# moberweger/deep-prior-pp

Measured on AMD Instinct MI355X. Metric: depth-crops/sec (NYU ResNet50 bs128) 1/2/4/8 GPU; mean 3D joint err (mm), higher is better.
Workload: dtype f32; 1 GPU; NYU posereg_embedding ResNet (type 0, 30-D PCA prior) train step: fused augment + fwd + bwd + ADAM, bs128/GPU fp32, 128x128x1 crops; global_batch=128, parallelism=dp1, augment=True, augment_pipelined=True, bn=local per-GPU batch statistics, launch_mode=native

## Files before the change

deep-prior-pp_amd/csrc/gemm_expand.hip:

```cpp
#include "gemm_args.h"

namespace {

template <int KT, bool BKC, bool IT2, bool ACT, bool RES, bool BNB, bool LZ = false, bool PB = false, bool ST = false>
__global__ __launch_bounds__(DPP_THREADS) DPP_WAVES_PER_EU(1, 2) void gemm_expand_kernel(GemmArgs ga, int rpw) {
    static_assert(!PB || ((KT % 32 == 0 || KT == 16) && !LZ), "bf16 MFMA operands: whole 32-deep steps, or K = 16 with a zero upper half");
    dpp_kernarg_warm<sizeof(GemmArgs)>();
    const dpp_gemm_desc& d = ga.d;
    constexpr int KL = KT / 4, KV = KL / 4;
    constexpr int RT = 2, RI = 16 * RT;
    const int lane = threadIdx.x & 63, l15 = lane & 15, kq = lane >> 4;
    const int NG = d.N >> 6, nblk = d.M / rpw;
    const int gw = blockIdx.x * 4 + (threadIdx.x >> 6);
    if (gw >= NG * nblk) return;
    const int cg = gw % NG, rblk = gw / NG;
    const int n0 = cg * 64 + 4 * l15;
    const int wrow0 = rblk * rpw, iters = rpw / RI;
    const dpp_epilogue& ep = d.epi;
    const int modeA = ACT ? d.actA.mode : 0;
    const bool relu_mask = BNB && ep.bn_relu != 0;
    const bool a16 = ST && !LZ && ga.shA != 0, c16 = ST && (d.store & DPP_ST_C) != 0, x16 = ST && (d.store & DPP_ST_BNX) != 0;
    dpp_stamp(ga.prof, 0);

    float bw[4][KL];
    if (BKC) {
#pragma unroll
        for (int ct = 0; ct < 4; ++ct)
#pragma unroll
            for (int j = 0; j < KV; ++j) {
                const float4 t = *reinterpret_cast<const float4*>(d.B + (size_t)(n0 + ct) * d.ldb + kq * KL + 4 * j);
                bw[ct][4 * j] = t.x; bw[ct][4 * j + 1] = t.y; bw[ct][4 * j + 2] = t.z; bw[ct][4 * j + 3] = t.w;
            }
    } else {
#pragma unroll
        for (int e = 0; e < KL; ++e) {
            const float4 t = *reinterpret_cast<const float4*>(d.B + (size_t)(kq * KL + e) * d.ldb + n0);
            bw[0][e] = t.x; bw[1][e] = t.y; bw[2][e] = t.z; bw[3][e] = t.w;
        }
    }
    constexpr int KS = PB ? (KL + 7) / 8 : 1;
    dpp_bf16x8 bwp[4][KS];
    if (PB) {
#pragma unroll
        for (int ct = 0; ct < 4; ++ct)
#pragma unroll
            for (int ss = 0; ss < KS; ++ss)
#pragma unroll
                for (int q = 0; q < 8; ++q) bwp[ct][ss][q] = (dpp_bf16)(ss * 8 + q < KL ? bw[ct][ss * 8 + q < KL ? ss * 8 + q : 0] : 0.0f);
    }
    struct Regs { float4 a[RT][KV]; float4 a2[RT][LZ ? KV : 1]; float4 res[RT][4]; float4 bx[RT][4]; };
    auto fetch = [&](Regs& g, int it) {
        const int r0 = wrow0 + it * RI;
#pragma unroll
        for (int rt = 0; rt < RT; ++rt) {
            const size_t oa = (size_t)(r0 + rt * 16 + l15) * d.lda + kq * KL;
            if (a16) {
#pragma unroll
                for (int j = 0; j < KV; ++j) g.a[rt][j] = dpp_raw8(d.A + ((oa + 4 * j) >> 1));
            } else {
#pragma unroll
                for (int j = 0; j < KV; ++j) {
                    g.a[rt][j] = *reinterpret_cast<const float4*>(d.A + oa + 4 * j);
                    if (LZ) g.a2[rt][j] = *reinterpret_cast<const float4*>(d.actA.x2 + oa + 4 * j);
                }
            }
        }
#pragma unroll
        for (int rt = 0; rt < RT; ++rt)
#pragma unroll
            for (int r = 0; r < 4; ++r) {
                const size_t o = (size_t)(r0 + rt * 16 + kq * 4 + r) * d.ldc + n0;
                if (RES) g.res[rt][r] = c16 ? dpp_raw8(d.residual + (o >> 1)) : *reinterpret_cast<const float4*>(d.residual + o);
                if (BNB) g.bx[rt][r] = x16 ? dpp_raw8(ep.bn_x + (o >> 1)) : *reinterpret_cast<const float4*>(ep.bn_x + o);
            }
    };
    Regs g0, g1;
    fetch(g0, 0);
    float4 mu[KV], sc[KV], be[KV], ax[LZ ? KV : 1];
#pragma unroll
    for (int j = 0; j < KV; ++j) {
        mu[j] = sc[j] = be[j] = make_float4(0.f, 0.f, 0.f, 0.f);
        if (LZ || (modeA & 2)) {
            mu[j] = *reinterpret_cast<const float4*>(d.actA.mean + kq * KL + 4 * j);
            sc[j] = *reinterpret_cast<const float4*>(d.actA.scale + kq * KL + 4 * j);
            be[j] = *reinterpret_cast<const float4*>(d.actA.beta + kq * KL + 4 * j);
        }
        if (LZ) ax[j] = *reinterpret_cast<const float4*>(d.actA.aux + kq * KL + 4 * j);
    }
    const bool lz_store = LZ && d.actA.out != nullptr && cg == 0;
    float4 cbias = make_float4(0.f, 0.f, 0.f, 0.f), cmean = cbias, cscale = cbias, cbeta = cbias, cistd = cbias;
    if (d.bias) cbias = *reinterpret_cast<const float4*>(d.bias + n0);
    if (BNB) {
        cmean = *reinterpret_cast<const float4*>(ep.bn_mean + n0); cscale = *reinterpret_cast<const float4*>(ep.bn_scale + n0);
        cbeta = *reinterpret_cast<const float4*>(ep.bn_beta + n0); cistd = *reinterpret_cast<const float4*>(ep.bn_inv_std + n0);
    }
    dpp_stamp(ga.prof, 1);

    float sx[4] = {0.f, 0.f, 0.f, 0.f}, sy[4] = {0.f, 0.f, 0.f, 0.f};
    float rmean[4] = {0.f, 0.f, 0.f, 0.f}, rm2[4] = {0.f, 0.f, 0.f, 0.f};
    const bool want_stats = ep.stats != nullptr;
    auto colsum = [&](float (&s)[4]) {
#pragma unroll
        for (int j = 0; j < 4; ++j) { s[j] += __shfl_xor(s[j], 16); s[j] += __shfl_xor(s[j], 32); }
    };

    auto step = [&](Regs& g, int it) {
        const int r0 = wrow0 + it * RI;
        f32x4 acc[RT][4];
#pragma unroll
        for (int rt = 0; rt < RT; ++rt)
#pragma unroll
            for (int ct = 0; ct < 4; ++ct) acc[rt][ct] = (f32x4){0.f, 0.f, 0.f, 0.f};
        dpp_bf16x8 ap[RT][KS];
        if (PB && KL < 8) {
#pragma unroll
            for (int rt = 0; rt < RT; ++rt)
#pragma unroll
                for (int q = 0; q < 8; ++q) ap[rt][0][q] = (dpp_bf16)0.0f;
        }
#pragma unroll
        for (int j = 0; j < KV; ++j) {
            float av[RT][4];
#pragma unroll
            for (int rt = 0; rt < RT; ++rt) {
                float4 v = a16 ? dpp_widen4(g.a[rt][j]) : g.a[rt][j];
                if (LZ) {
                    const float4 x = g.a2[rt][j];
                    v = make_float4(sc[j].x * v.x - ax[j].x * (x.x - mu[j].x) - be[j].x, sc[j].y * v.y - ax[j].y * (x.y - mu[j].y) - be[j].y,
                                    sc[j].z * v.z - ax[j].z * (x.z - mu[j].z) - be[j].z, sc[j].w * v.w - ax[j].w * (x.w - mu[j].w) - be[j].w);
                    if (lz_store) *reinterpret_cast<float4*>(d.actA.out + (size_t)(r0 + rt * 16 + l15) * d.lda + kq * KL + 4 * j) = v;
                }
                if (modeA & 2) {
                    v.x = dpp_fma(v.x - mu[j].x, sc[j].x, be[j].x); v.y = dpp_fma(v.y - mu[j].y, sc[j].y, be[j].y);
                    v.z = dpp_fma(v.z - mu[j].z, sc[j].z, be[j].z); v.w = dpp_fma(v.w - mu[j].w, sc[j].w, be[j].w);
                }
                if (modeA & 1) { v.x = fmaxf(v.x, 0.f); v.y = fmaxf(v.y, 0.f); v.z = fmaxf(v.z, 0.f); v.w = fmaxf(v.w, 0.f); }
                av[rt][0] = v.x; av[rt][1] = v.y; av[rt][2] = v.z; av[rt][3] = v.w;
                if (PB) {
#pragma unroll
                    for (int t = 0; t < 4; ++t) ap[rt][j / 2][(j & 1) * 4 + t] = (dpp_bf16)av[rt][t];
                }
            }
            if (PB) {
                if ((j & 1) || KL < 8) {
#pragma unroll
                    for (int rt = 0; rt < RT; ++rt)
#pragma unroll
                        for (int ct = 0; ct < 4; ++ct)
                            acc[rt][ct] = __builtin_amdgcn_mfma_f32_16x16x32_bf16(ap[rt][j / 2], bwp[ct][j / 2], acc[rt][ct], 0, 0, 0);
                }
            } else {
#pragma unroll
                for (int t = 0; t < 4; ++t)
#pragma unroll
                    for (int rt = 0; rt < RT; ++rt)
#pragma unroll
                        for (int ct = 0; ct < 4; ++ct)
                            acc[rt][ct] = __builtin_amdgcn_mfma_f32_16x16x4f32(av[rt][t], bw[ct][4 * j + t], acc[rt][ct], 0, 0, 0);
            }
        }
        float vals[RT][4][4];
#pragma unroll
        for (int rt = 0; rt < RT; ++rt)
#pragma unroll
            for (int r = 0; r < 4; ++r) {
                float v[4] = {acc[rt][0][r] + cbias.x, acc[rt][1][r] + cbias.y, acc[rt][2][r] + cbias.z, acc[rt][3][r] + cbias.w};
                if (RES) {
                    const float4 rr = c16 ? dpp_widen4(g.res[rt][r]) : g.res[rt][r];
                    v[0] += rr.x; v[1] += rr.y; v[2] += rr.z; v[3] += rr.w;
                }
                if (BNB) {
                    const float4 bxv = x16 ? dpp_widen4(g.bx[rt][r]) : g.bx[rt][r];
                    const float x[4] = {bxv.x, bxv.y, bxv.z, bxv.w};
                    const float cm[4] = {cmean.x, cmean.y, cmean.z, cmean.w}, cs[4] = {cscale.x, cscale.y, cscale.z, cscale.w};
                    const float cb[4] = {cbeta.x, cbeta.y, cbeta.z, cbeta.w}, ci[4] = {cistd.x, cistd.y, cistd.z, cistd.w};
#pragma unroll
                    for (int j = 0; j < 4; ++j) {
                        const float dx = x[j] - cm[j];
                        if (relu_mask && dx * cs[j] + cb[j] < 0.0f) v[j] = 0.0f;
                        if (c16) v[j] = dpp_bf16_round(v[j]);
                        sx[j] += v[j];
                        sy[j] += v[j] * (dx * ci[j]);
                    }
                }
                {
                    const size_t oc = (size_t)(r0 + rt * 16 + kq * 4 + r) * d.ldc + n0;
                    if (c16) dpp_st4(reinterpret_cast<dpp_bf16*>(d.C) + oc, make_float4(v[0], v[1], v[2], v[3]));
                    else *reinterpret_cast<float4*>(d.C + oc) = make_float4(v[0], v[1], v[2], v[3]);
                }
#pragma unroll
                for (int j = 0; j < 4; ++j) vals[rt][r][j] = v[j];
            }
        if (want_stats) {
            float sm[4] = {0.f, 0.f, 0.f, 0.f}, m2[4] = {0.f, 0.f, 0.f, 0.f};
#pragma unroll
            for (int rt = 0; rt < RT; ++rt)
#pragma unroll
                for (int r = 0; r < 4; ++r)
#pragma unroll
                    for (int j = 0; j < 4; ++j) sm[j] += vals[rt][r][j];
            colsum(sm);
#pragma unroll
            for (int j = 0; j < 4; ++j) sm[j] *= 1.0f / (float)RI;
#pragma unroll
            for (int rt = 0; rt < RT; ++rt)
#pragma unroll
                for (int r = 0; r < 4; ++r)
#pragma unroll
                    for (int j = 0; j < 4; ++j) { const float dv = vals[rt][r][j] - sm[j]; m2[j] += dv * dv; }
            colsum(m2);
            if (it == 0) {
#pragma unroll
                for (int j = 0; j < 4; ++j) { rmean[j] = sm[j]; rm2[j] = m2[j]; }
            } else {
                const float na = (float)(it * RI), nb = (float)RI, nn = na + nb;
#pragma unroll
                for (int j = 0; j < 4; ++j) {
                    const float dl = sm[j] - rmean[j];
                    rmean[j] += dl * (nb / nn);
                    rm2[j] += m2[j] + dl * dl * (na * nb / nn);
                }
            }
        }
    };

    if (IT2) {
        for (int it = 0; it < iters; it += 2) {
            if (it + 1 < iters) fetch(g1, it + 1);
            DPP_SCHED_FENCE();
            step(g0, it);
            if (it + 1 < iters) {
                if (it + 2 < iters) fetch(g0, it + 2);
                DPP_SCHED_FENCE();
                step(g1, it + 1);
            }
        }
    } else {
        DPP_SCHED_FENCE();
        step(g0, 0);
    }
    dpp_stamp(ga.prof, 3);
    if (BNB && ep.bn_partial != nullptr) {
        float tx[4] = {sx[0], sx[1], sx[2], sx[3]}, ty[4] = {sy[0], sy[1], sy[2], sy[3]};
        colsum(tx);
        colsum(ty);
        if (kq == 0) {
#pragma unroll
            for (int j = 0; j < 4; ++j) {
                ep.bn_partial[dpp_partial_index(0, n0 + j, rblk, d.N, nblk)] = tx[j];
                ep.bn_partial[dpp_partial_index(1, n0 + j, rblk, d.N, nblk)] = ty[j];
            }
        }
    }
    if (want_stats && kq == 0) {
#pragma unroll
        for (int j = 0; j < 4; ++j) {
            ep.stats[dpp_partial_index(0, n0 + j, rblk, d.N, nblk)] = rmean[j];
            ep.stats[dpp_partial_index(1, n0 + j, rblk, d.N, nblk)] = rm2[j];
        }
    }
    dpp_stamp(ga.prof, 4);
}

}

int dpp_gemm_expand_rows(const dpp_gemm_desc& d, const GemmArgs& ga) {
    if ((d.store & DPP_ST_B) || (d.store && (d.actA.mode & 4))) return 0;
    if (!d.a_kc || d.splitk != 1 || !d.C || !ga.vecA || !ga.vecB || !ga.wide) return 0;
    if (d.K != 16 && d.K != 32 && d.K != 64) return 0;
    if (d.N % 64 || d.M % 32) return 0;
    if (d.mapA.s != 1 || d.mapB.s != 1 || d.mapC.s != 1 || d.actB.mode != 0) return 0;
    if (d.actA.mode != 0 && d.actA.cmod < d.K) return 0;
    if (d.epi.stats && d.epi.bn_x) return 0;
    if (d.b_kc ? (d.epi.bn_x != nullptr || (d.actA.mode & 4)) : (d.actA.mode != 0 && d.actA.mode != 4)) return 0;
    if (d.actA.mode == 4 && d.actA.out && d.lda != d.K) return 0;
    if (d.precision != 0 && (d.precision != 1 || (d.actA.mode & 4))) return 0;
    int rpw = d.bm;
    if (rpw <= 0) rpw = d.M >= 65536 ? 128 : (d.M >= 16384 ? 64 : 32);
    if (rpw % 32 || d.M % rpw) return 0;
    return rpw;
}

namespace {

template <int KT>
int launch_expand(const GemmArgs& ga, int rpw, hipStream_t st) {
    const dpp_gemm_desc& d = ga.d;
    const int waves = (d.M / rpw) * (d.N / 64);
    const dim3 grid(dpp_cdiv(waves, 4));
    const bool it2 = rpw > 32, act = d.actA.mode != 0, res = d.residual != nullptr, bnb = d.epi.bn_x != nullptr, lz = d.actA.mode == 4;
    const bool pb = d.precision == 1;
    const bool stg = d.store != 0;
#define DPP_EXS(K_, I_, A_, R_, B_, L_, P_, S_) DPP_LAUNCH((gemm_expand_kernel<KT, K_, I_, A_, R_, B_, L_, P_, S_>), grid, dim3(DPP_THREADS), 0, st, ga, rpw)
#define DPP_EX(K_, I_, A_, R_, B_, L_, P_) do { if (!(L_) && stg) DPP_EXS(K_, I_, A_, R_, B_, L_, P_, !(L_)); else DPP_EXS(K_, I_, A_, R_, B_, L_, P_, false); } while (0)
#define DPP_EX_P(K_, I_, A_, R_, B_) do { if (pb) { DPP_EX(K_, I_, A_, R_, B_, false, true); break; } \
                                          DPP_EX(K_, I_, A_, R_, B_, false, false); } while (0)
#define DPP_EX_I(K_, A_, R_, B_, L_) do { if (L_) { if (it2) DPP_EX(K_, true, A_, R_, B_, true, false); else DPP_EX(K_, false, A_, R_, B_, true, false); } \
                                          else if (it2) DPP_EX_P(K_, true, A_, R_, B_); else DPP_EX_P(K_, false, A_, R_, B_); } while (0)
#define DPP_EX_R(K_, A_, B_, L_) do { if (res) DPP_EX_I(K_, A_, true, B_, L_); else DPP_EX_I(K_, A_, false, B_, L_); } while (0)
    if (d.b_kc) {
        if (act) DPP_EX_R(true, true, false, false); else DPP_EX_R(true, false, false, false);
    } else if (lz) {
        if (bnb) DPP_EX_R(false, false, true, true); else DPP_EX_R(false, false, false, true);
    } else {
        if (bnb) DPP_EX_R(false, false, true, false); else DPP_EX_R(false, false, false, false);
    }
#undef DPP_EX_P
#undef DPP_EXS
#undef DPP_EX_R
#undef DPP_EX_I
#undef DPP_EX
    return dpp_launch_status();
}

}

int dpp_gemm_expand_launch(const GemmArgs& ga, int rpw, hipStream_t st) {
    const dpp_gemm_desc& d = ga.d;
    return d.K == 64 ? launch_expand<64>(ga, rpw, st) : (d.K == 32 ? launch_expand<32>(ga, rpw, st) : launch_expand<16>(ga, rpw, st));
}
```

Baseline: 38050 depth-crops/sec.

## Share expand-GEMM filter slice across block waves via LDS with XCD-aware block remap

In the 1x1 expand GEMM, the four waves of a block now share one 64-column filter slice. Each thread loads a piece of the slice cooperatively into LDS, and each wave then reads its register image from LDS instead of every wave loading the whole slice from global memory. Block indices are optionally remapped so that blocks on the same XCD handle the same column group, which should improve L2 reuse of B. The path is on by default, is gated on shape conditions with an env override, and excludes a few configurations. It adds an LDS barrier and LDS traffic at kernel start.

```diff
diff --git a/deep-prior-pp_amd/csrc/gemm_expand.hip b/deep-prior-pp_amd/csrc/gemm_expand.hip
--- a/deep-prior-pp_amd/csrc/gemm_expand.hip
+++ b/deep-prior-pp_amd/csrc/gemm_expand.hip
@@ -1,9 +1,18 @@
 #include "gemm_args.h"
+#include <cstdlib>
+
+#ifdef DPP_HIP_EMU
+#define DPP_LDS_BARRIER() __syncthreads()
+#else
+#define DPP_LDS_BARRIER() do { __builtin_amdgcn_fence(__ATOMIC_RELEASE, "workgroup", "local"); __builtin_amdgcn_s_barrier(); \
+                               __builtin_amdgcn_fence(__ATOMIC_ACQUIRE, "workgroup", "local"); } while (0)
+#endif
 
 namespace {
 
-template <int KT, bool BKC, bool IT2, bool ACT, bool RES, bool BNB, bool LZ = false, bool PB = false, bool ST = false>
-__global__ __launch_bounds__(DPP_THREADS) DPP_WAVES_PER_EU(1, 2) void gemm_expand_kernel(GemmArgs ga, int rpw) {
+template <int KT, bool BKC, bool IT2, bool ACT, bool RES, bool BNB, bool LZ = false, bool PB = false, bool ST = false, bool SH = false>
+__global__ __launch_bounds__(DPP_THREADS) DPP_WAVES_PER_EU(1, 2) void gemm_expand_kernel(GemmArgs ga, int rpw, int xcd) {
+    static_assert(!SH || KT >= 32, "the shared filter slice: K = 32 / 64 (whole 256-thread passes over the slice)");
     static_assert(!PB || ((KT % 32 == 0 || KT == 16) && !LZ), "bf16 MFMA operands: whole 32-deep steps, or K = 16 with a zero upper half");
     dpp_kernarg_warm<sizeof(GemmArgs)>();
     const dpp_gemm_desc& d = ga.d;
@@ -11,9 +20,18 @@
     constexpr int RT = 2, RI = 16 * RT;
     const int lane = threadIdx.x & 63, l15 = lane & 15, kq = lane >> 4;
     const int NG = d.N >> 6, nblk = d.M / rpw;
-    const int gw = blockIdx.x * 4 + (threadIdx.x >> 6);
-    if (gw >= NG * nblk) return;
-    const int cg = gw % NG, rblk = gw / NG;
+    int cg, rblk;
+    if (SH) {
+        int v = blockIdx.x;
+        if (xcd) v = (v & 7) * ((int)gridDim.x >> 3) + (v >> 3);
+        cg = v % NG;
+        rblk = 4 * (v / NG) + (threadIdx.x >> 6);
+    } else {
+        const int gw = blockIdx.x * 4 + (threadIdx.x >> 6);
+        if (gw >= NG * nblk) return;
+        cg = gw % NG;
+        rblk = gw / NG;
+    }
     const int n0 = cg * 64 + 4 * l15;
     const int wrow0 = rblk * rpw, iters = rpw / RI;
     const dpp_epilogue& ep = d.epi;
@@ -23,7 +41,40 @@
     dpp_stamp(ga.prof, 0);
 
     float bw[4][KL];
-    if (BKC) {
+    constexpr int KS = PB ? (KL + 7) / 8 : 1;
+    dpp_bf16x8 bwp[4][KS];
+    auto pack_bw = [&]() {
+        if (PB) {
+#pragma unroll
+            for (int ct = 0; ct < 4; ++ct)
+#pragma unroll
+                for (int ss = 0; ss < KS; ++ss)
+#pragma unroll
+                    for (int q = 0; q < 8; ++q) bwp[ct][ss][q] = (dpp_bf16)(ss * 8 + q < KL ? bw[ct][ss * 8 + q < KL ? ss * 8 + q : 0] : 0.0f);
+        }
+    };
+    float4 bp0, bp1, bp2, bp3;
+    int bs0 = 0, bs1 = 0, bs2 = 0, bs3 = 0;
+    auto bpiece = [&](int i, float4& v, int& slot) {
+        if (BKC) {
+            const int wi = (threadIdx.x >> 6) + 4 * i;
+            const int o = wi & 7, ln = wi >> 3;
+            const int bl15 = 8 * (o >> 2) + ((lane >> 2) & 7), bct = o & 3;
+            const int kp = 8 * ln + 4 * (lane >> 5) + (lane & 3);
+            v = *reinterpret_cast<const float4*>(d.B + (size_t)(cg * 64 + 4 * bl15 + bct) * d.ldb + 4 * kp);
+            slot = (bct * KV + kp % KV) * 64 + (kp / KV) * 16 + bl15;
+        } else {
+            const int p = threadIdx.x + DPP_THREADS * i, k = p >> 4, c = p & 15;
+            v = *reinterpret_cast<const float4*>(d.B + (size_t)k * d.ldb + cg * 64 + 4 * c);
+            slot = (k % KL) * 64 + (k / KL) * 16 + c;
+        }
+    };
+    if (SH) {
+        bpiece(0, bp0, bs0);
+        bpiece(1, bp1, bs1);
+        if (KV > 2) { bpiece(2, bp2, bs2); bpiece(3, bp3, bs3); }
+        DPP_SCHED_FENCE();
+    } else if (BKC) {
 #pragma unroll
         for (int ct = 0; ct < 4; ++ct)
 #pragma unroll
@@ -38,16 +89,7 @@
             bw[0][e] = t.x; bw[1][e] = t.y; bw[2][e] = t.z; bw[3][e] = t.w;
         }
     }
-    constexpr int KS = PB ? (KL + 7) / 8 : 1;
-    dpp_bf16x8 bwp[4][KS];
-    if (PB) {
-#pragma unroll
-        for (int ct = 0; ct < 4; ++ct)
-#pragma unroll
-            for (int ss = 0; ss < KS; ++ss)
-#pragma unroll
-                for (int q = 0; q < 8; ++q) bwp[ct][ss][q] = (dpp_bf16)(ss * 8 + q < KL ? bw[ct][ss * 8 + q < KL ? ss * 8 + q : 0] : 0.0f);
-    }
+    if (!SH) pack_bw();
     struct Regs { float4 a[RT][KV]; float4 a2[RT][LZ ? KV : 1]; float4 res[RT][4]; float4 bx[RT][4]; };
     auto fetch = [&](Regs& g, int it) {
         const int r0 = wrow0 + it * RI;
@@ -93,6 +135,20 @@
     if (BNB) {
         cmean = *reinterpret_cast<const float4*>(ep.bn_mean + n0); cscale = *reinterpret_cast<const float4*>(ep.bn_scale + n0);
         cbeta = *reinterpret_cast<const float4*>(ep.bn_beta + n0); cistd = *reinterpret_cast<const float4*>(ep.bn_inv_std + n0);
+    }
+    if constexpr (SH) {
+        __shared__ float4 bimg[KT * 16];
+        bimg[bs0] = bp0;
+        bimg[bs1] = bp1;
+        if (KV > 2) { bimg[bs2] = bp2; bimg[bs3] = bp3; }
+        DPP_LDS_BARRIER();
+#pragma unroll
+        for (int q = 0; q < KL; ++q) {
+            const float4 t = bimg[q * 64 + lane];
+            if (BKC) { bw[q / KV][4 * (q % KV)] = t.x; bw[q / KV][4 * (q % KV) + 1] = t.y; bw[q / KV][4 * (q % KV) + 2] = t.z; bw[q / KV][4 * (q % KV) + 3] = t.w; }
+            else { bw[0][q] = t.x; bw[1][q] = t.y; bw[2][q] = t.z; bw[3][q] = t.w; }
+        }
+        pack_bw();
     }
     dpp_stamp(ga.prof, 1);
 
@@ -291,7 +347,16 @@
     const bool it2 = rpw > 32, act = d.actA.mode != 0, res = d.residual != nullptr, bnb = d.epi.bn_x != nullptr, lz = d.actA.mode == 4;
     const bool pb = d.precision == 1;
     const bool stg = d.store != 0;
-#define DPP_EXS(K_, I_, A_, R_, B_, L_, P_, S_) DPP_LAUNCH((gemm_expand_kernel<KT, K_, I_, A_, R_, B_, L_, P_, S_>), grid, dim3(DPP_THREADS), 0, st, ga, rpw)
+    const char* se = getenv("DPP_EXPAND_SHARE");
+    const int share = se ? atoi(se) : 1;
+    const bool can = KT != 16 && d.M % (4 * rpw) == 0 && (!d.b_kc || d.ldb == d.K);
+    const bool faster = !(it2 && ((KT == 32 && !d.b_kc && (res || lz)) || (KT == 64 && lz)));
+    const bool sh = share != 0 && can && (faster || share == 3);
+    const int ng = d.N / 64, xcd = sh && share != 2 && grid.x % 8 == 0 && (grid.x / 8) % ng == 0;
+    if (getenv("DPP_EXPAND_SHARE_VERBOSE")) fprintf(stderr, "gemm_expand_kernel: K %d N %d M %d rpw %d: %s\n", d.K, d.N, d.M, rpw, sh ? "shared filter slice" : "wave-autonomous");
+#define DPP_EXS(K_, I_, A_, R_, B_, L_, P_, S_) do { \
+        if (sh) DPP_LAUNCH((gemm_expand_kernel<KT, K_, I_, A_, R_, B_, L_, P_, S_, KT != 16>), grid, dim3(DPP_THREADS), 0, st, ga, rpw, xcd); \
+        else DPP_LAUNCH((gemm_expand_kernel<KT, K_, I_, A_, R_, B_, L_, P_, S_, false>), grid, dim3(DPP_THREADS), 0, st, ga, rpw, 0); } while (0)
 #define DPP_EX(K_, I_, A_, R_, B_, L_, P_) do { if (!(L_) && stg) DPP_EXS(K_, I_, A_, R_, B_, L_, P_, !(L_)); else DPP_EXS(K_, I_, A_, R_, B_, L_, P_, false); } while (0)
 #define DPP_EX_P(K_, I_, A_, R_, B_) do { if (pb) { DPP_EX(K_, I_, A_, R_, B_, false, true); break; } \
                                           DPP_EX(K_, I_, A_, R_, B_, false, false); } while (0)
```

Result: no change. 38350 depth-crops/sec, median of 6 (+0.8%).
